# fskovbo/OptimalControlMPS

Measured on NVIDIA B200. Metric: cost+gradient evals/s (BH N=20 chi=100), higher is better.
Workload: dtype complex128 (f64)

## Files before the change

### optimalcontrolmps_b200/csrc/decomp.cu

```cuda
#include <cstdio>
#include <cstdlib>
#include "ocmps_internal.h"

__device__ unsigned long long g_jac_dbg[8];
__device__ double g_jac_flops[2];

namespace {

constexpr int JAC_THREADS = 512;
constexpr int JAC_EPL = 8;
constexpr int JAC_NV_SMEM = 512;
constexpr int JAC_MAX_SWEEPS = 60;
constexpr int JAC_BLOCKED_ROWS = 64;
constexpr double JAC_TOL2 = 1e-28;
constexpr double DEFLATE_REL = 1e-30;
constexpr int NV_MAX = 2048;
constexpr int BJ_C = 8;
constexpr int BJ_TPP = 4;
constexpr int BJ_MAX_ROWS = 256;
constexpr int BJ_SLOTS = BJ_MAX_ROWS / 2;
constexpr int BJ_THREADS = BJ_SLOTS * BJ_TPP;
constexpr int BJ_MAX_EPL = 8;
constexpr int BJ_MIN_CAP = 112;

// ... 987 lines not shown
    hF[blockIdx.x] = F;
    hK[blockIdx.x] = keff;
    hB[blockIdx.x] = -1;
    hS[blockIdx.x] = ldz;
    const double nn = (double)len, mmv = (double)nv;
    atomicAdd(&g_jac_flops[0], 8.0 * nn * nn * mmv + (56.0 / 3.0) * nn * nn * nn);
    if (blockIdx.x == 0) {
      const double dn = mode == 0 ? (double)w->n : (double)w->m, dm = mode == 0 ? (double)w->m : (double)w->n;
      atomicAdd(&g_jac_flops[1], 8.0 * dn * dn * dm + (56.0 / 3.0) * dn * dn * dn);
    }
    if (nv >= 64) {
      const long long t_now = clock64();
      atomicAdd(&g_jac_dbg[5], (unsigned long long)(t_now - t_qr0));
      atomicAdd(&g_jac_dbg[7], (unsigned long long)(t_now - t_start));
#ifdef OCMPS_JAC_TRACE
      printf("JTG kind %d blk %d nv %d len %d keff %d gather+gram %lld cholesky+out %lld\n", a.kind, (int)blockIdx.x, nv, len, keff,
             (long long)(t_qr0 - t_start), (long long)(t_now - t_qr0));
#endif
    }
  }
  return true;
}

__global__ void __launch_bounds__(JAC_THREADS) jacobi_rot_kernel(DecompArgs a, DecompBuffers b, int smem_elems) {
  extern __shared__ __align__(16) unsigned char smem_raw[];
  __shared__ int s_rot, s_big;
  __shared__ double s_nrm[JAC_BLOCKED_ROWS];
  const DecompWork* w = b.dw;
  if ((int)blockIdx.x >= w->nblocks) return;
  {
    const int nv0 = w->blk[blockIdx.x].nv, len0 = w->blk[blockIdx.x].len;
    const bool fits = nv0 * len0 <= smem_elems && nv0 <= JAC_NV_SMEM;
    const int ldpad = ((nv0 + 15) >> 4) << 4;
    const bool can_cache = nv0 <= 16 * JAC_EPL && (nv0 < len0 ? nv0 : len0) * ldpad <= smem_elems;
    if (!(fits && can_cache)) return;
  }
  const int keff = reinterpret_cast<const int*>(b.scratch_d + 7 * NV_MAX + OCMPS_MAX_BLK)[blockIdx.x];
  if (keff < 0) return;
  const DecompBlock B = w->blk[blockIdx.x];
  const int nv = B.nv;
  const int tid = threadIdx.x, lane = tid & 31, warp = tid >> 5, nwarps = JAC_THREADS / 32;
  const int epl = (nv + 15) >> 4, ldz = epl << 4;
  const double F = (b.scratch_d + 7 * NV_MAX)[blockIdx.x];
  const double thr = F * DEFLATE_REL;
  const short* perm = reinterpret_cast<const short*>(b.scratch_d + 4 * NV_MAX) + B.p_off;
  cplx* Ya = b.ywork + B.ws_off;
  const cplx* Yb = b.ywork + b.ywork_half + B.ws_off;
  cplx* Z = reinterpret_cast<cplx*>(smem_raw);
  double* nrm = s_nrm;
  const long long t_jac0 = clock64();
  for (int e = tid; e < keff * ldz; e += JAC_THREADS) Z[e] = Yb[e];
  __syncthreads();
  bool converged = false;
  for (int sweep = 0; sweep < JAC_MAX_SWEEPS && !converged; ++sweep) {
    for (int v = warp; v < keff; v += nwarps) {
      const cplx* y = Z + v * ldz;
      double s = 0.0;
      for (int c = lane; c < nv; c += 32) { cplx u = y[c]; s += u.x * u.x + u.y * u.y; }
      s = warp_sum(s);
      if (lane == 0) nrm[v] = s;
    }
    if (tid == 0) { s_rot = 0; s_big = 0; }
    __syncthreads();
    if (keff < 2) break;
    switch (epl) {
      case 1: jacobi_sweep_blocked<1>(Z, keff, nrm, thr, &s_rot, &s_big); break;
      case 2: jacobi_sweep_blocked<2>(Z, keff, nrm, thr, &s_rot, &s_big); break;
      case 3: jacobi_sweep_blocked<3>(Z, keff, nrm, thr, &s_rot, &s_big); break;
      case 4: jacobi_sweep_blocked<4>(Z, keff, nrm, thr, &s_rot, &s_big); break;
      case 5: jacobi_sweep_blocked<5>(Z, keff, nrm, thr, &s_rot, &s_big); break;
      case 6: jacobi_sweep_blocked<6>(Z, keff, nrm, thr, &s_rot, &s_big); break;
      case 7: jacobi_sweep_blocked<7>(Z, keff, nrm, thr, &s_rot, &s_big); break;
      default: jacobi_sweep_blocked<8>(Z, keff, nrm, thr, &s_rot, &s_big); break;
    }
    converged = (s_rot == 0) || (s_big == 0);
    if (tid == 0) { atomicAdd(&g_jac_dbg[0], 1ull); atomicMax(&g_jac_dbg[2], (unsigned long long)(sweep + 1)); if (nv >= 64) atomicAdd(&g_jac_dbg[3], 1ull); if (nv >= 64 && sweep == 0) atomicAdd(&g_jac_dbg[4], 1ull); }
    __syncthreads();
    if (!converged && sweep == JAC_MAX_SWEEPS - 1 && tid == 0) atomicOr(b.status, OCMPS_ST_NOCONV);
  }
  __syncthreads();
  const long long t_jac1 = clock64();
  if (tid == 0) {
    atomicAdd(&g_jac_dbg[1], 1ull);
    if (nv >= 64) {
      atomicAdd(&g_jac_dbg[6], (unsigned long long)(t_jac1 - t_jac0));
      atomicAdd(&g_jac_dbg[7], (unsigned long long)(t_jac1 - t_jac0));
    }
#ifdef OCMPS_JAC_TRACE
    if (nv >= 24) printf("JT2 kind %d blk %d nv %d keff %d jac %lld\n", a.kind, (int)blockIdx.x, nv, keff, t_jac1 - t_jac0);
#endif
  }
  for (int v = warp; v < nv; v += nwarps) {
    if (v < keff) {
      const cplx* y = Z + v * ldz;
      double s = 0.0;
      for (int c = lane; c < nv; c += 32) { cplx u = y[c]; s += u.x * u.x + u.y * u.y; }
      s = warp_sum(s);
      const double inv = s > 0.0 ? rsqrt(s) : 0.0;
      for (int c = lane; c < nv; c += 32) {
        cplx u = y[c];
        Ya[v * nv + (int)perm[c]] = make_double2(u.x * inv, u.y * inv);
      }
      if (lane == 0) b.P[B.p_off + v] = s;
    } else if (lane == 0) {
      b.P[B.p_off + v] = 0.0;
    }
  }
}

namespace clus {
__device__ __forceinline__ unsigned smem_u32(const void* p) { return (unsigned)__cvta_generic_to_shared(p); }
__device__ __forceinline__ unsigned mapa(unsigned addr, unsigned rank) {
  unsigned r;
  asm volatile("mapa.shared::cluster.u32 %0, %1, %2;" : "=r"(r) : "r"(addr), "r"(rank));
  return r;
}
__device__ __forceinline__ void st_async_v2(unsigned raddr, double a, double b, unsigned rmbar) {
  asm volatile("st.async.weak.shared::cluster.mbarrier::complete_tx::bytes.v2.f64 [%0], {%1, %2}, [%3];" ::"r"(raddr), "d"(a), "d"(b), "r"(rmbar) : "memory");
}
__device__ __forceinline__ void mbar_init(unsigned mbar, unsigned count) { asm volatile("mbarrier.init.shared::cta.b64 [%0], %1;" ::"r"(mbar), "r"(count) : "memory"); }
__device__ __forceinline__ void mbar_expect(unsigned mbar, unsigned bytes) {
  asm volatile("mbarrier.arrive.expect_tx.shared::cta.b64 _, [%0], %1;" ::"r"(mbar), "r"(bytes) : "memory");
}
__device__ __forceinline__ void mbar_wait(unsigned mbar, unsigned parity) {
  asm volatile(
      "{\n.reg .pred p;\nWAIT_%=:\n"
      "mbarrier.try_wait.parity.shared::cta.b64 p, [%0], %1;\n"
      "@p bra DONE_%=;\nbra WAIT_%=;\nDONE_%=:\n}\n" ::"r"(mbar), "r"(parity) : "memory");
}
__device__ __forceinline__ void cluster_sync() { asm volatile("barrier.cluster.arrive.release.aligned;\nbarrier.cluster.wait.acquire.aligned;\n" ::: "memory"); }
// ... 488 lines not shown
      case 3: bj_run<8, 3>(b, B, keff, ldz, F, Rs, sh); break;
      default: bj_run<8, 4>(b, B, keff, ldz, F, Rs, sh); break;
    }
  } else {
    switch ((wcols + 3) / 4) {
      case 1: bj_run<4, 1>(b, B, keff, ldz, F, Rs, sh); break;
      case 2: bj_run<4, 2>(b, B, keff, ldz, F, Rs, sh); break;
      case 3: bj_run<4, 3>(b, B, keff, ldz, F, Rs, sh); break;
      case 4: bj_run<4, 4>(b, B, keff, ldz, F, Rs, sh); break;
      case 5: bj_run<4, 5>(b, B, keff, ldz, F, Rs, sh); break;
      case 6: bj_run<4, 6>(b, B, keff, ldz, F, Rs, sh); break;
      case 7: bj_run<4, 7>(b, B, keff, ldz, F, Rs, sh); break;
      default: bj_run<4, 8>(b, B, keff, ldz, F, Rs, sh); break;
    }
  }
  clus::cluster_sync();
  if (tid == 0 && clus::cluster_rank() == 0) {
    atomicAdd(&g_jac_dbg[1], 1ull);
    const long long t1 = clock64();
    if (B.nv >= 64) { atomicAdd(&g_jac_dbg[6], (unsigned long long)(t1 - t0)); atomicAdd(&g_jac_dbg[7], (unsigned long long)(t1 - t0)); }
#ifdef OCMPS_JAC_TRACE
    if (B.nv >= 24) printf("JT3 kind %d blk %d nv %d keff %d jac %lld\n", a.kind, blk, B.nv, keff, (long long)(t1 - t0));
#endif
  }
}

__global__ void __launch_bounds__(1024) truncate_kernel(DecompArgs a, DecompBuffers b, TruncParams tp) {
  __shared__ double cP[NV_MAX];
  __shared__ double sSorted[NV_MAX];
  __shared__ short cQ[NV_MAX], cI[NV_MAX], cI2[NV_MAX];
  __shared__ unsigned char sKeep[NV_MAX];
  __shared__ int sBlkOff[OCMPS_MAX_BLK + 1];
  __shared__ double sWarp[32];
  __shared__ int sWarpCnt[33];
  __shared__ double s_docut, s_kept;
  __shared__ int s_nfinal;
  DecompWork* w = b.dw;
  const int nv = w->nvtot;
  const int nblocks = w->nblocks;
  const int tid = threadIdx.x, lane = tid & 31, warp = tid >> 5;
  for (int i = tid; i < nblocks; i += blockDim.x) sBlkOff[i] = w->blk[i].p_off;
  if (tid == 0) { s_nfinal = 0; s_docut = 0.0; }
  const int i0 = 2 * tid, i1 = i0 + 1;
  const double p0 = i0 < nv ? b.P[i0] : 0.0, p1 = i1 < nv ? b.P[i1] : 0.0;
  const int f0 = p0 > 0.0, f1 = p1 > 0.0;
  int incl = f0 + f1;
// ... 366 lines not shown
    x[e] = make_double2(u.x * inv, u.y * inv);
  }
}
__global__ void norm_finish_kernel(const double* partial, double* out) {
  if (threadIdx.x == 0 && blockIdx.x == 0) *out = sqrt(norm_total(partial));
}

int grid_for(long long elems, int threads, int cap = 1184) {
  long long g = (elems + threads - 1) / threads;
  if (g < 1) g = 1;
  if (g > cap) g = cap;
  return (int)g;
}

}

static bool g_jac_attr_set[64] = {false};

void debug_jacobi_counters(unsigned long long* out, bool reset) {
  cudaMemcpyFromSymbol(out, g_jac_dbg, sizeof(unsigned long long) * 8);
  if (reset) { unsigned long long z[8] = {0}; cudaMemcpyToSymbol(g_jac_dbg, z, sizeof(z)); }
}

__global__ void __launch_bounds__(256) spectrum_entropy_kernel(DecompBuffers b, double* out) {
  __shared__ double red[256];
  const int nv = b.dw->nvtot;
  double acc = 0.0;
  for (int i = threadIdx.x; i < nv; i += 256) {
    const double p = b.P[i];
    if (p > 1e-12) acc -= p * log(p);
  }
  red[threadIdx.x] = acc;
  __syncthreads();
  for (int o = 128; o > 0; o >>= 1) {
    if ((int)threadIdx.x < o) red[threadIdx.x] += red[threadIdx.x + o];
    __syncthreads();
  }
  if (threadIdx.x == 0) *out = red[0];
}

void launch_spectrum_entropy(const DecompBuffers& b, double* out, cudaStream_t s) {
  spectrum_entropy_kernel<<<1, 256, 0, s>>>(b, out);
}

void launch_decomp_setup(const DecompArgs& a, const DecompBuffers& b, cudaStream_t s) {
  decomp_setup_kernel<<<1, SETUP_THREADS, 0, s>>>(a, b);
// ... 7 lines not shown

bool profile_is_on() { return g_prof_on; }

void profile_enable(bool on) {
  g_prof_on = on;
  g_prof_used = 0;
  double z[2] = {0.0, 0.0};
  cudaMemcpyToSymbol(g_jac_flops, z, sizeof(z));
}
void profile_read(double* out) {
  cudaDeviceSynchronize();
  double ms = 0.0;
  for (size_t i = 0; i < g_prof_used; ++i) {
    float t = 0.f;
    cudaEventElapsedTime(&t, g_prof_events[i].first, g_prof_events[i].second);
    ms += t;
  }
  double fl[2];
  cudaMemcpyFromSymbol(fl, g_jac_flops, sizeof(fl));
  out[0] = ms; out[1] = (double)g_prof_used; out[2] = fl[0]; out[3] = fl[1];
}

void launch_jacobi_blocks(const DecompArgs& a, const DecompBuffers& b, int nblk_launch, size_t smem_limit, bool need_global,
                          bool long_rows, double rank_tol, int max_rows, int capV, int capC, cudaStream_t s, const SvdFork* fork) {
  cudaEvent_t e0 = nullptr, e1 = nullptr;
  if (g_prof_on) {
    if (g_prof_used == g_prof_events.size()) {
      cudaEvent_t x, y;
      cudaEventCreate(&x); cudaEventCreate(&y);
      g_prof_events.push_back({x, y});
    }
    e0 = g_prof_events[g_prof_used].first; e1 = g_prof_events[g_prof_used].second;
    ++g_prof_used;
    cudaEventRecord(e0, s);
  }
  struct Tail { cudaEvent_t e; cudaStream_t s; ~Tail() { if (e) cudaEventRecord(e, s); } } tail{e1, s};
  int dev = 0;
  cudaGetDevice(&dev);
  static std::mutex attr_mu;
  if (dev < 64) {
  std::lock_guard<std::mutex> attr_lock(attr_mu);
  if (!g_jac_attr_set[dev]) {
    cudaFuncSetAttribute(jacobi_blocks_kernel<true, true>, cudaFuncAttributeMaxDynamicSharedMemorySize, 200 * 1024);
    cudaFuncSetAttribute(jacobi_blocks_kernel<true, false>, cudaFuncAttributeMaxDynamicSharedMemorySize, 200 * 1024);
    cudaFuncSetAttribute(build_factors_kernel, cudaFuncAttributeMaxDynamicSharedMemorySize, 96 * 1024);
    cudaFuncSetAttribute(jacobi_rot_kernel, cudaFuncAttributeMaxDynamicSharedMemorySize, (int)(JAC_BLOCKED_ROWS * 16 * JAC_EPL * sizeof(cplx)));
    cudaFuncSetAttribute(jacobi_big_kernel, cudaFuncAttributeMaxDynamicSharedMemorySize, (int)(BJ_MAX_ROWS * (BJ_TPP * BJ_MAX_EPL + 4) * sizeof(cplx)));
    cudaFuncSetAttribute(qr_big_kernel, cudaFuncAttributeMaxDynamicSharedMemorySize, (int)((32 * BJ_MAX_ROWS + BJ_MAX_ROWS) * sizeof(cplx)));
    g_jac_attr_set[dev] = true;
  }
  }
  static const bool big_env = [] { const char* e = getenv("OCMPS_BIG_CLUSTER"); return !(e && e[0] == '0'); }();
  int big_on = (big_env && max_rows >= BJ_MIN_CAP) ? 1 : 0;
  static const bool gram_env = [] { const char* e = getenv("OCMPS_GRAM"); return e && e[0] == '1'; }();
  if (gram_env && (a.kind == DK_GATE_LEFT || a.kind == DK_GATE_RIGHT)) big_on |= 2;
  static const bool fork_env = [] { const char* e = getenv("OCMPS_SVD_FORK"); return !(e && e[0] == '0'); }();
  const bool forked = fork_env && (big_on & 1) && fork && fork->stream;
  cudaStream_t sb = forked ? fork->stream : s;
  if (forked) { cudaEventRecord(fork->ev_fork, s); cudaStreamWaitEvent(sb, fork->ev_fork, 0); }
  jacobi_blocks_kernel<true, true><<<nblk_launch, JAC_THREADS, smem_limit, s>>>(a, b, (int)(smem_limit / sizeof(cplx)), rank_tol, big_on);
  if (forked) cudaEventRecord(fork->ev_first, s);
  if (long_rows) jacobi_blocks_kernel<true, false><<<nblk_launch, JAC_THREADS, smem_limit, s>>>(a, b, (int)(smem_limit / sizeof(cplx)), rank_tol, big_on);
  if (need_global) jacobi_blocks_kernel<false, false><<<nblk_launch, JAC_THREADS, 0, s>>>(a, b, (int)(smem_limit / sizeof(cplx)), rank_tol, big_on);
  if (big_on & 1) {
    cudaLaunchConfig_t cfg = {};
    cfg.gridDim = dim3(nblk_launch * BJ_C, 1, 1);
    cfg.blockDim = dim3(BJ_THREADS, 1, 1);
    cfg.dynamicSmemBytes = (size_t)(32 * BJ_MAX_ROWS + BJ_MAX_ROWS) * sizeof(cplx);
    cfg.stream = sb;
    cudaLaunchAttribute at[1];
    at[0].id = cudaLaunchAttributeClusterDimension;
    at[0].val.clusterDim.x = BJ_C; at[0].val.clusterDim.y = 1; at[0].val.clusterDim.z = 1;
    cfg.attrs = at; cfg.numAttrs = 1;
    cudaLaunchKernelEx(&cfg, qr_big_kernel, a, b, (int)(smem_limit / sizeof(cplx)), rank_tol);
  }
  jacobi_rot_kernel<<<nblk_launch, JAC_THREADS, JAC_BLOCKED_ROWS * 16 * JAC_EPL * sizeof(cplx), s>>>(a, b, (int)(smem_limit / sizeof(cplx)));
  if (big_on & 1) {
    if (forked) cudaStreamWaitEvent(sb, fork->ev_first, 0);
    cudaLaunchConfig_t cfg = {};
    cfg.gridDim = dim3(nblk_launch * BJ_C, 1, 1);
    cfg.blockDim = dim3(BJ_THREADS, 1, 1);
    cfg.dynamicSmemBytes = (size_t)BJ_MAX_ROWS * (BJ_TPP * BJ_MAX_EPL + 4) * sizeof(cplx);
    cfg.stream = sb;
    cudaLaunchAttribute at[1];
    at[0].id = cudaLaunchAttributeClusterDimension;
    at[0].val.clusterDim.x = BJ_C; at[0].val.clusterDim.y = 1; at[0].val.clusterDim.z = 1;
    cfg.attrs = at; cfg.numAttrs = 1;
    cudaLaunchKernelEx(&cfg, jacobi_big_kernel, a, b);
    if (forked) { cudaEventRecord(fork->ev_join, sb); cudaStreamWaitEvent(s, fork->ev_join, 0); }
  }
}

void launch_truncate(const DecompArgs& a, const DecompBuffers& b, const TruncParams& tp, cudaStream_t s) {
  truncate_kernel<<<1, 1024, 0, s>>>(a, b, tp);
}

void launch_build_factors(const DecompArgs& a, const DecompBuffers& b, int cap_k, int cap_vec, int cap_comp, cudaStream_t s) {
  const size_t sm = (sizeof(cplx) + sizeof(int)) * (size_t)(cap_vec + cap_comp);
  build_factors_kernel<<<cap_k, BUILD_THREADS, sm, s>>>(a, b);
// ... 14 lines not shown
```

### optimalcontrolmps_b200/csrc/engine.cu

```cuda
#include <cmath>
#include <complex>
#include <cstdio>
#include <cstring>
#include <cstdlib>
#include <algorithm>
#include <string>
#include <atomic>
#include <chrono>
#include <map>
#include <mutex>
#include <tuple>
#include <thread>
#include <vector>

#include "ocmps_internal.h"
#include "../../include/ocmps.h"

std::atomic<long long> g_ocmps_launches{0};

namespace {

thread_local std::string g_err;

int fail(int code, const std::string& msg) {
// ... 84 lines not shown
struct Op {
  int kind;
  int a, b, c;
};

}

struct Workspace {
  ocmps_ctx* ctx = nullptr;
  int L = 0, D = 0, cap = 0;
  bool busy = false;
  size_t dead_seen = 0;
  int* d_status = nullptr;
  cplx* d_div = nullptr; int div_cap = 0;
  cudaStream_t stream = nullptr;
  cudaStream_t ovl = nullptr;
  cplx* theta = nullptr;
  cplx* cbuf = nullptr;
  DecompBuffers db;
  DecompBuffers db2;
  cudaStream_t side = nullptr;
  cudaEvent_t ev_trunc = nullptr, ev_setup = nullptr;
  SvdFork fork;
  cplx* E[2] = {nullptr, nullptr};
  cplx* T = nullptr;
  GemmDesc* odescs = nullptr;
  cplx* d_out = nullptr;
  int obatch = 0;
  long long e_stride = 0, t_stride = 0;
  ocmps_mps* work = nullptr;
  ocmps_mps* big = nullptr;
  Workspace* bigws = nullptr;
  double* d_norm = nullptr;
  StepParams* d_params = nullptr;
  ocmps_mps* tmpK = nullptr;
  ocmps_mps* psiH = nullptr;
  ocmps_store* rowstore = nullptr;
  struct StepGraph { cudaGraphExec_t exec = nullptr; unsigned long long flips = 0; int launches = 0; int seen = 0; };
  std::map<std::tuple<long long, long long, unsigned long long, int, int>, StepGraph> graphs;
};

struct ocmps_stepper {
  ocmps_ctx* ctx = nullptr;
  int L = 0, D = 0, cap = 0;
  double J = 1.0, tstep = 0.0;
  bool has_cutoff = false, has_maxm = false;
  double cutoff = MIN_CUT;
  int maxm = MAX_M;
  int rel_cutoff = 0;
  cplx* d_G[2] = {nullptr, nullptr};
  std::vector<std::complex<double>> h_G[2];
  std::vector<Op> ops;
  long long serial = 0;
  bool imag = false;
};

namespace {

int alloc_mps(ocmps_ctx* ctx, int L, int D, int cap, ocmps_mps** out, int mult = 1) {
  if (L < 1 || L > OCMPS_MAX_L) return fail(OCMPS_ERR_INVALID, "L out of range [1,64]");
  if (D < 2 || D > OCMPS_MAX_D) return fail(OCMPS_ERR_INVALID, "D out of range [2,8]");
  if (cap < 1 || (long long)cap * mult * D > NV_MAX) return fail(OCMPS_ERR_INVALID, "chi_cap*D exceeds 2048");
// ... 133 lines not shown
  void release() {
    if (!ctx || ws.empty()) return;
    std::lock_guard<std::mutex> lock(ctx->mu);
    for (Workspace* w : ws) w->busy = false;
    ws.clear();
  }
  int acquire(ocmps_ctx* c, int L, int D, int cap, int n) {
    ctx = c;
    std::lock_guard<std::mutex> lock(c->mu);
    for (Workspace* w : c->pool) {
      if ((int)ws.size() == n) break;
      if (!w->busy && w->L == L && w->D == D && w->cap == cap) { w->busy = true; ws.push_back(w); }
    }
    while ((int)ws.size() < n) {
      Workspace* w = nullptr;
      int same = 0;
      for (Workspace* o : c->pool) if (o->L == L && o->D == D && o->cap == cap) ++same;
      int rc = alloc_ws(c, L, D, cap, true, &w, same < 2);
      if (rc) return rc;
      w->busy = true;
      c->pool.push_back(w);
      ws.push_back(w);
    }
    for (Workspace* w : ws) {
      if (w->dead_seen == c->dead_mps.size()) continue;
      if (!w->graphs.empty()) {
        std::vector<long long> dead(c->dead_mps.begin() + w->dead_seen, c->dead_mps.end());
        std::sort(dead.begin(), dead.end());
        for (auto it = w->graphs.begin(); it != w->graphs.end();) {
          if (std::binary_search(dead.begin(), dead.end(), std::get<1>(it->first))) {
            if (it->second.exec) cudaGraphExecDestroy(it->second.exec);
            it = w->graphs.erase(it);
          } else {
            ++it;
          }
        }
      }
      w->dead_seen = c->dead_mps.size();
    }
    return OCMPS_OK;
  }
  Workspace* operator[](int i) const { return ws[i]; }
  int finish() {
    int st = 0;
    for (Workspace* w : ws) {
      CK(cudaStreamSynchronize(w->stream));
// ... 122 lines not shown
};
static StepTrace g_trace;
static bool step_trace_enabled() {
  static const bool v = [] { const char* e = getenv("OCMPS_STEP_TRACE"); return e && e[0] == '1'; }();
  return v;
}
enum { TR_START = 0, TR_MERGE, TR_SETUP, TR_SVD_GATE, TR_SVD_ORTH, TR_TRUNC, TR_BUILD, TR_OTHER, TR_NPHASE };

void run_decomp(Workspace* ws, const DecompArgs& a, const TruncParams& tp, int capV, int capC, int capK, cudaStream_t s,
                DecompBuffers* dbp = nullptr, bool setup_done = false, const DecompArgs* next = nullptr, DecompBuffers* db_next = nullptr) {
  DecompBuffers& db = dbp ? *dbp : ws->db;
  if (!setup_done) { launch_decomp_setup(a, db, s); g_trace.mark(TR_SETUP, s); }
  size_t need = (size_t)capV * capC * sizeof(cplx);
  need = std::max(need, (size_t)std::min(capV, capC) * (size_t)(((capV + 15) / 16) * 16) * sizeof(cplx));
  size_t smem = std::min(need, JAC_SMEM_LIMIT);
  if (smem < 1024) smem = 1024;
  int nblk = std::min(std::min(OCMPS_MAX_BLK, std::max(capV, capC) + a.D), ws->ctx->qmax.load() + a.D + 1);
  const bool need_global = need > JAC_SMEM_LIMIT;
  static const double rank_scale = [] { const char* e = getenv("OCMPS_RANK_TOL_SCALE"); return e ? atof(e) : 1e-6; }();
  double rank_tol = rank_scale * tp.cutoff;
  rank_tol = std::min(rank_scale * 1e-8, std::max(1e-30, rank_tol));
  const bool long_rows = capV > 128;
  const int max_rows = std::min(capV, capC);
  launch_jacobi_blocks(a, db, nblk, smem, need_global, long_rows, rank_tol, max_rows, capV, capC, s, &ws->fork);
  g_trace.mark((a.kind == DK_GATE_LEFT || a.kind == DK_GATE_RIGHT) ? TR_SVD_GATE : TR_SVD_ORTH, s);
  launch_truncate(a, db, tp, s);
  g_trace.mark(TR_TRUNC, s);
  if (next) {
    cudaEventRecord(ws->ev_trunc, s);
    cudaStreamWaitEvent(ws->side, ws->ev_trunc, 0);
    launch_decomp_setup(*next, *db_next, ws->side);
    cudaEventRecord(ws->ev_setup, ws->side);
  }
  launch_build_factors(a, db, capK, capV, capC, s);
  g_trace.mark(TR_BUILD, s);
  g_ocmps_launches += 5 + (need_global ? 1 : 0) + (long_rows ? 1 : 0);
}

void phases_of(int D, double U, double tstep, double* re, double* im, bool imag = false) {
  for (int n = 0; n < D; ++n) {
    if (imag) {
      re[n] = std::exp(-0.25 * U * tstep * (double)n * (double)(n - 1));
      im[n] = 0.0;
      continue;
    }
    const double ang = -0.25 * U * tstep * (double)n * (double)(n - 1);
    re[n] = std::cos(ang);
// ... 172 lines not shown
    g_trace.on = false;
    CK(cudaStreamSynchronize(s));
    double sum[TR_NPHASE] = {0};
    int cnt[TR_NPHASE] = {0};
    for (size_t i = 1; i < g_trace.marks.size(); ++i) {
      float ms = 0.f;
      cudaEventElapsedTime(&ms, g_trace.marks[i - 1].second, g_trace.marks[i].second);
      sum[g_trace.marks[i].first] += ms;
      ++cnt[g_trace.marks[i].first];
    }
    float tot = 0.f;
    cudaEventElapsedTime(&tot, g_trace.marks.front().second, g_trace.marks.back().second);
    static const char* names[TR_NPHASE] = {"", "merge_gate", "setup", "svd(gate)", "svd(gauge)", "truncate", "build", "other"};
    fprintf(stderr, "[ocmps step] %.3f ms:", tot);
    for (int p = 1; p < TR_NPHASE; ++p) fprintf(stderr, " %s %dx %.3f |", names[p], cnt[p], sum[p]);
    fprintf(stderr, "\n");
    for (auto& m2 : g_trace.marks) cudaEventDestroy(m2.second);
    g_trace.marks.clear();
    return OCMPS_OK;
  }
  if (!graphs_enabled() || profile_is_on()) { body(); return OCMPS_OK; }
  unsigned long long parity = 0;
  for (int j = 0; j < lay.L; ++j) parity |= (unsigned long long)(m->cur[j] & 1) << j;
  auto key = std::make_tuple(st->serial, m->serial, parity, store ? 1 : 0, ws->ctx->qmax.load());
  Workspace::StepGraph& g = ws->graphs[key];
  if (g.exec) {
    for (int j = 0; j < lay.L; ++j) m->cur[j] ^= (int)((g.flips >> j) & 1ull);
    m->llim = 0; m->rlim = 2;
    g_ocmps_launches += g.launches;
    CK(cudaGraphLaunch(g.exec, s));
    return OCMPS_OK;
  }
  if (g.seen == 0) {
    g.seen = 1;
    body();
    return OCMPS_OK;
  }
  if (ws->graphs.size() > 64) {
    for (auto& kv : ws->graphs) if (kv.second.exec) cudaGraphExecDestroy(kv.second.exec);
    ws->graphs.clear();
    Workspace::StepGraph& g2 = ws->graphs[key];
    g2.seen = 1;
    body();
    return OCMPS_OK;
  }
  const long long l0 = g_ocmps_launches;
  cudaGraph_t graph = nullptr;
// ... 89 lines not shown
                                        int qstride_out, int L, int cap_out, int* status) {
  for (int b = blockIdx.x; b <= L; b += gridDim.x) {
    int d = dims_in[b];
    if (d > cap_out) { if (threadIdx.x == 0) atomicOr(status, OCMPS_ST_CAPACITY); d = cap_out; }
    if (threadIdx.x == 0) dims_out[b] = d;
    for (int i = threadIdx.x; i < d; i += blockDim.x) q_out[(size_t)b * qstride_out + i] = q_in[(size_t)b * qstride_in + i];
  }
}

int apply_K_async(ocmps_stepper* st, Workspace* ws, ocmps_mps* in, ocmps_mps* out, cudaStream_t s) {
  const int L = st->L, D = st->D;
  const int cap2 = 2 * st->cap;
  if ((long long)cap2 * D > NV_MAX) return fail(OCMPS_ERR_INVALID, "apply_K: 2*chi_cap*D exceeds 2048");
  if (!ws->big) {
    int rc = alloc_mps(st->ctx, L, D, st->cap, &ws->big, 2);
    if (rc) return rc;
    rc = alloc_ws(st->ctx, L, D, cap2, false, &ws->bigws);
    if (rc) return rc;
    ws->bigws->db.status = ws->d_status;
    ws->bigws->db2.status = ws->d_status;
  }
  ocmps_mps* big = ws->big;
  Workspace* bw = ws->bigws;
  const Layout& lb = big->lay;
  if (L == 1) return fail(OCMPS_ERR_INVALID, "apply_K needs L >= 2");
  for (int j = 0; j < L; ++j) big->cur[j] = 0;
  for (int j = 0; j < L; ++j) {
    launch_applyK_expand(in->site(j), big->site(j), in->dim(j), in->dim(j + 1), in->q(j), in->q(j + 1), big->dim(j), big->dim(j + 1),
                         big->q(j), big->q(j + 1), D, j, L, lb.capb[j] * D * lb.capb[j + 1], s);
  }
  g_ocmps_launches += L;
  TruncParams tpl{MIN_CUT, MAX_M, 1, 1, 0, 0};
  for (int b = 1; b <= L - 1; ++b) {
    const int j = b - 1, jn = b;
    DecompArgs a;
    a.D = D; a.kind = DK_ORTH_LEFT;
    a.dimNew = big->dim(b); a.qNew = big->q(b); a.partner = bw->cbuf;
    a.dimL = big->dim(b - 1); a.dimR = big->dim(b); a.qL = big->q(b - 1); a.qR = big->q(b);
    a.X = big->site(j); a.iso = big->other(j);
    a.nb_in = big->site(jn); a.nb_out = big->other(jn); a.dimNb = big->dim(b + 1);
    a.qNb = fused_push_enabled() ? big->q(b + 1) : nullptr;
    tpl.cap = lb.capb[b];
    run_decomp(bw, a, tpl, lb.capb[b], lb.capb[b - 1], lb.capb[b], s);
    if (!a.qNb) launch_zgemm(bw->db.descs + 1, 1, lb.capb[b], D * lb.capb[b + 1], s);
    big->cur[j] ^= 1; big->cur[jn] ^= 1;
    g_ocmps_launches += 1;
// ... 341 lines not shown

static int check_shapes(ocmps_stepper* st, const Layout& lay, const char* what) {
  if (lay.L != st->L || lay.D != st->D || lay.cap != st->cap)
    return fail(OCMPS_ERR_INVALID, std::string(what) + ": MPS/store shape (L, D, chi_cap) differs from the stepper's");
  return OCMPS_OK;
}

int ocmps_step(ocmps_stepper* st, ocmps_mps* psi, double from, double to, int forward) {
  if (!st || !psi) return fail(OCMPS_ERR_INVALID, "null argument");
  int rc = check_shapes(st, psi->lay, "step");
  if (rc) return rc;
  if (psi->llim != 0 || psi->rlim != 2) return fail(OCMPS_ERR_INVALID, "step: orthogonality centre must be at site 1");
  CK(cudaSetDevice(st->ctx->dev));
  WsLease lease;
  rc = lease.acquire(st->ctx, st->L, st->D, st->cap, 1);
  if (rc) return rc;
  Workspace* ws = lease[0];
  rc = step_enqueue(st, psi, ws, from, to, forward != 0, nullptr, 0, ws->stream);
  if (rc) { cudaStreamSynchronize(ws->stream); return rc; }
  return lease.finish();
}

int ocmps_debug_jacobi(unsigned long long* out, int reset) { cudaDeviceSynchronize(); debug_jacobi_counters(out, reset != 0); return 0; }

int ocmps_debug_run_ops(ocmps_stepper* st, ocmps_mps* psi, double from, double to, int forward, int op_begin, int op_end) {
  CK(cudaSetDevice(st->ctx->dev));
  WsLease lease;
  int rc = lease.acquire(st->ctx, st->L, st->D, st->cap, 1);
  if (rc) return rc;
  Workspace* ws = lease[0];
  { StepParams hp; fill_step_params(st, from, to, forward != 0, nullptr, 0, hp); launch_set_step_params(hp, ws->d_params, ws->stream); }
  run_step_body(st, psi, ws, ws->stream, op_begin, op_end);
  return lease.finish();
}

int ocmps_apply_K(ocmps_stepper* st, ocmps_mps* in, ocmps_mps* out) {
  if (!st || !in || !out) return fail(OCMPS_ERR_INVALID, "null argument");
  int rc = check_shapes(st, in->lay, "apply_K");
  if (rc) return rc;
  rc = check_shapes(st, out->lay, "apply_K");
  if (rc) return rc;
  CK(cudaSetDevice(st->ctx->dev));
  WsLease lease;
  rc = lease.acquire(st->ctx, st->L, st->D, st->cap, 1);
  if (rc) return rc;
  Workspace* ws = lease[0];
// ... 814 lines not shown
```

### optimalcontrolmps_b200/csrc/ocmps_internal.h

```cpp
#pragma once
#include <cuda_runtime.h>
#include <stdint.h>
#include <stddef.h>

typedef double2 cplx;

#define OCMPS_MAX_L 64
#define OCMPS_MAX_D 8
#define OCMPS_MAX_Q 256
#define OCMPS_MAX_BLK 128

#define OCMPS_ST_CAPACITY   1
#define OCMPS_ST_NOCONV     2
#define OCMPS_ST_CHARGE     4
#define OCMPS_ST_TOOMANYBLK 8

struct GemmDesc {
  const cplx* A; const cplx* B; cplx* C;
  int M, N, K;
  int lda, ldb, ldc;
  int opA, opB;
  int pad;
};

// ... 19 lines not shown
  double cutoff;
  int maxm, minm;
  int rel_cutoff;
  int cap;
  int normalize;
};

struct StepParams {
  double u1r[OCMPS_MAX_D], u1i[OCMPS_MAX_D];
  double u2r[OCMPS_MAX_D], u2i[OCMPS_MAX_D];
  const cplx* G;
  cplx* slot_data; int* slot_dims; int* slot_q;
};

struct SitePtrs { cplx* p[OCMPS_MAX_L]; };
struct SiteOffs { long long o[OCMPS_MAX_L + 1]; };

struct Phases { double re[4][OCMPS_MAX_D]; double im[4][OCMPS_MAX_D]; };

#include <atomic>
extern std::atomic<long long> g_ocmps_launches;

void debug_jacobi_counters(unsigned long long* out, bool reset);
void profile_enable(bool on);
bool profile_is_on();
void profile_read(double* out);

void launch_zgemm(const GemmDesc* d_descs, int batch, int maxM, int maxN, cudaStream_t s);

enum DecompKind { DK_GATE_LEFT = 0, DK_GATE_RIGHT = 1, DK_ORTH_LEFT = 2, DK_ORTH_RIGHT = 3 };

struct DecompArgs {
  int kind;
  int D;
  const int* dimL;
  const int* dimR;
  const int* qL;
  const int* qR;
  int* dimNew;
  int* qNew;
  const cplx* X;
  cplx* iso;
  cplx* partner;
  const cplx* nb_in;
  cplx* nb_out;
  const int* dimNb;
  const int* qNb;
};

struct DecompBuffers {
  DecompWork* dw;
  int* vec_idx; int* comp_idx;
  int* vecq;
  double* P;
  int* pos;
  cplx* ywork;
  long long ywork_half;
  double* scratch_d;
  GemmDesc* descs;
  double* partial;
  int* status;
};

void launch_decomp_setup(const DecompArgs& a, const DecompBuffers& b, cudaStream_t s);
struct SvdFork { cudaStream_t stream = nullptr; cudaEvent_t ev_fork = nullptr, ev_first = nullptr, ev_join = nullptr; };
void launch_jacobi_blocks(const DecompArgs& a, const DecompBuffers& b, int nblk_launch, size_t smem_limit, bool need_global,
                          bool long_rows, double rank_tol, int max_rows, int capV, int capC, cudaStream_t s, const SvdFork* fork = nullptr);
void launch_spectrum_entropy(const DecompBuffers& b, double* out, cudaStream_t s);
void launch_truncate(const DecompArgs& a, const DecompBuffers& b, const TruncParams& tp, cudaStream_t s);
void launch_build_factors(const DecompArgs& a, const DecompBuffers& b, int cap_k, int cap_vec, int cap_comp, cudaStream_t s);

void launch_merge_setup(GemmDesc* d, const cplx* A1, const cplx* A2, cplx* theta, const int* dimL, const int* dimM,
                        const int* dimR, int D, cudaStream_t s);
void launch_merge_gate(const cplx* A1, const cplx* A2, cplx* theta, const int* dimL, const int* dimM, const int* dimR,
                       const int* qL, const int* qM, const int* qR, int D, const StepParams* sp, int gate_kind, int maxL, int maxR,
                       cudaStream_t s);
void launch_gate_apply(cplx* theta, const int* dimL, const int* dimR, const int* qL, const int* qR, int D, const StepParams* sp,
                       int gate_kind, int maxL, int maxR, cudaStream_t s);
void launch_site_phase(cplx* A, const int* dimL, const int* dimR, int D, const StepParams* sp, int which, int max_elems, cudaStream_t s);
void launch_set_step_params(const StepParams& hp, StepParams* dst, cudaStream_t s);
void launch_pack_to_slot(SitePtrs src, SiteOffs offs, const int* dims, const int* q, int L, int D, int cap, int max_site_elems,
                         const StepParams* sp, int* status, cudaStream_t s);
void launch_norm_only(const cplx* x, const int* dimL, const int* dimR, int D, double* partial, double* out, int max_elems,
                      cudaStream_t s);
void launch_normalize_site(cplx* x, const int* dimL, const int* dimR, int D, double* partial, int max_elems, cudaStream_t s);

void launch_pack_copy(SitePtrs src, cplx* dst_base, SiteOffs offs, const int* dims, int L, int D, int max_site_elems, int* status,
                      cudaStream_t s);
void launch_unpack_copy(const cplx* src_base, SitePtrs dst, SiteOffs offs, const int* dims, int L, int D, int max_site_elems, int* status,
                        cudaStream_t s);
// ... 26 lines not shown
```

Before: 0.8572.

## Spread one-sided Jacobi rows across a 4-CTA cluster with DSMEM block exchange

Adds a cluster kernel that splits the Jacobi rotation of a symmetry block across four CTAs. Each CTA holds two row blocks and runs round-robin block pairs, exchanging row blocks and norms through distributed shared memory between rounds, and combines convergence flags across the cluster. It is enabled when the workspace batch is small (n<=2), so the GPU is underused and a single CTA per block is the bottleneck. The cost is a cluster sync and a DSMEM copy every round. Blocks with fewer than 40 effective rows fall back to the single-CTA path.

```diff
diff --git a/optimalcontrolmps_b200/csrc/decomp.cu b/optimalcontrolmps_b200/csrc/decomp.cu
--- a/optimalcontrolmps_b200/csrc/decomp.cu
+++ b/optimalcontrolmps_b200/csrc/decomp.cu
@@ -1033,26 +1033,26 @@
   return true;
 }
 
-__global__ void __launch_bounds__(JAC_THREADS) jacobi_rot_kernel(DecompArgs a, DecompBuffers b, int smem_elems) {
-  extern __shared__ __align__(16) unsigned char smem_raw[];
+__device__ __forceinline__ int rot_handover_rows(const DecompBuffers& b, int blk, int smem_elems) {
+  const DecompWork* w = b.dw;
+  if (blk >= w->nblocks) return -1;
+  const int nv0 = w->blk[blk].nv, len0 = w->blk[blk].len;
+  const bool fits = nv0 * len0 <= smem_elems && nv0 <= JAC_NV_SMEM;
+  const int ldpad = ((nv0 + 15) >> 4) << 4;
+  const bool can_cache = nv0 <= 16 * JAC_EPL && (nv0 < len0 ? nv0 : len0) * ldpad <= smem_elems;
+  if (!(fits && can_cache)) return -1;
+  return reinterpret_cast<const int*>(b.scratch_d + 7 * NV_MAX + OCMPS_MAX_BLK)[blk];
+}
+
+__device__ __forceinline__ void jacobi_rot_block(const DecompArgs& a, const DecompBuffers& b, int blk, int keff, unsigned char* smem_raw) {
   __shared__ int s_rot, s_big;
   __shared__ double s_nrm[JAC_BLOCKED_ROWS];
   const DecompWork* w = b.dw;
-  if ((int)blockIdx.x >= w->nblocks) return;
-  {
-    const int nv0 = w->blk[blockIdx.x].nv, len0 = w->blk[blockIdx.x].len;
-    const bool fits = nv0 * len0 <= smem_elems && nv0 <= JAC_NV_SMEM;
-    const int ldpad = ((nv0 + 15) >> 4) << 4;
-    const bool can_cache = nv0 <= 16 * JAC_EPL && (nv0 < len0 ? nv0 : len0) * ldpad <= smem_elems;
-    if (!(fits && can_cache)) return;
-  }
-  const int keff = reinterpret_cast<const int*>(b.scratch_d + 7 * NV_MAX + OCMPS_MAX_BLK)[blockIdx.x];
-  if (keff < 0) return;
-  const DecompBlock B = w->blk[blockIdx.x];
+  const DecompBlock B = w->blk[blk];
   const int nv = B.nv;
   const int tid = threadIdx.x, lane = tid & 31, warp = tid >> 5, nwarps = JAC_THREADS / 32;
   const int epl = (nv + 15) >> 4, ldz = epl << 4;
-  const double F = (b.scratch_d + 7 * NV_MAX)[blockIdx.x];
+  const double F = (b.scratch_d + 7 * NV_MAX)[blk];
   const double thr = F * DEFLATE_REL;
   const short* perm = reinterpret_cast<const short*>(b.scratch_d + 4 * NV_MAX) + B.p_off;
   cplx* Ya = b.ywork + B.ws_off;
@@ -1098,7 +1098,7 @@
       atomicAdd(&g_jac_dbg[7], (unsigned long long)(t_jac1 - t_jac0));
     }
 #ifdef OCMPS_JAC_TRACE
-    if (nv >= 24) printf("JT2 kind %d blk %d nv %d keff %d jac %lld\n", a.kind, (int)blockIdx.x, nv, keff, t_jac1 - t_jac0);
+    if (nv >= 24) printf("JT2 kind %d blk %d nv %d keff %d jac %lld\n", a.kind, blk, nv, keff, t_jac1 - t_jac0);
 #endif
   }
   for (int v = warp; v < nv; v += nwarps) {
@@ -1117,6 +1117,13 @@
       b.P[B.p_off + v] = 0.0;
     }
   }
+}
+
+__global__ void __launch_bounds__(JAC_THREADS) jacobi_rot_kernel(DecompArgs a, DecompBuffers b, int smem_elems) {
+  extern __shared__ __align__(16) unsigned char smem_raw[];
+  const int keff = rot_handover_rows(b, (int)blockIdx.x, smem_elems);
+  if (keff < 0) return;
+  jacobi_rot_block(a, b, (int)blockIdx.x, keff, smem_raw);
 }
 
 namespace clus {
@@ -1651,6 +1658,238 @@
 #ifdef OCMPS_JAC_TRACE
     if (B.nv >= 24) printf("JT3 kind %d blk %d nv %d keff %d jac %lld\n", a.kind, blk, B.nv, keff, (long long)(t1 - t0));
 #endif
+  }
+}
+
+constexpr int RC_C = 4;
+constexpr int RC_NBLK = 2 * RC_C;
+constexpr int RC_ROWS = JAC_BLOCKED_ROWS / RC_NBLK;
+constexpr int RC_WORK_THREADS = 16 * RC_ROWS;
+constexpr int RC_MIN_ROWS = 40;
+
+__device__ unsigned long long g_rc_dbg[2];
+
+struct RcShared {
+  double nrm[2][2][RC_ROWS];
+  int flags[2][RC_C];
+  int rot, big;
+};
+
+__device__ __forceinline__ void rc_blocks(int R, int s, int& P, int& Q) {
+  constexpr int mm = RC_NBLK - 1;
+  int p = R + s; if (p >= mm) p -= mm;
+  int q = R - s; if (q < 0) q += mm;
+  if (s == 0) q = RC_NBLK - 1;
+  P = p; Q = q;
+}
+
+__device__ __forceinline__ void rc_bar() { asm volatile("bar.sync 1, %0;" ::"n"(RC_WORK_THREADS) : "memory"); }
+
+template <int EPL>
+__device__ __forceinline__ void rc_block_round(cplx* __restrict__ Z0, cplx* __restrict__ Z1, double* n0, double* n1, int rb, int base0, int base1,
+                                               int keff, double thr, bool intra, int* s_rot, int* s_big) {
+  constexpr int ldz = 16 * EPL;
+  const int tid = threadIdx.x, hl = tid & 15, h = tid >> 4;
+  cplx ra[EPL], rb_[EPL];
+  double na = 0.0, nb = 0.0;
+  auto load_row = [&](cplx (&r)[EPL], double& n, const cplx* Z, const double* nz, int row) {
+    const cplx* z = Z + (row >= 0 ? row : 0) * ldz + hl;
+#pragma unroll
+    for (int e = 0; e < EPL; ++e) r[e] = row >= 0 ? z[16 * e] : make_double2(0.0, 0.0);
+    n = row >= 0 ? nz[row] : 0.0;
+  };
+  auto store_row = [&](const cplx (&r)[EPL], double n, cplx* Z, double* nz, int row) {
+    cplx* z = Z + row * ldz + hl;
+#pragma unroll
+    for (int e = 0; e < EPL; ++e) z[16 * e] = r[e];
+    if (hl == 0) nz[row] = n;
+  };
+  if (intra) {
+    const int X = h / (RC_ROWS / 2), j = h % (RC_ROWS / 2);
+    cplx* Z = X ? Z1 : Z0;
+    double* nz = X ? n1 : n0;
+    const int base = X ? base1 : base0;
+    const int rbp = (rb + 1) & ~1, m = rbp - 1;
+    for (int r = 0; r < m; ++r) {
+      int p = r + j; if (p >= m) p -= m;
+      int q = r - j; if (q < 0) q += m;
+      if (j == 0) q = m;
+      const bool act = 2 * j < rbp && p < rb && q < rb && base + p < keff && base + q < keff;
+      load_row(ra, na, Z, nz, act ? p : -1);
+      load_row(rb_, nb, Z, nz, act ? q : -1);
+      jac_rotate<EPL>(ra, rb_, na, nb, act, thr, hl, s_rot, s_big);
+      if (act) { store_row(ra, na, Z, nz, p); store_row(rb_, nb, Z, nz, q); }
+      rc_bar();
+    }
+  }
+  const bool has_a = h < rb && base0 + h < keff;
+  load_row(ra, na, Z0, n0, has_a ? h : -1);
+  for (int t = 0; t < rb; ++t) {
+    int jb = h + t; if (jb >= rb) jb -= rb;
+    const bool act = has_a && base1 + jb < keff;
+    load_row(rb_, nb, Z1, n1, act ? jb : -1);
+    jac_rotate<EPL>(ra, rb_, na, nb, act, thr, hl, s_rot, s_big);
+    if (act) store_row(rb_, nb, Z1, n1, jb);
+    rc_bar();
+  }
+  if (has_a) store_row(ra, na, Z0, n0, h);
+}
+
+template <int EPL>
+__device__ __forceinline__ void rc_run(const DecompArgs& a, const DecompBuffers& b, int blk, int keff, unsigned rank, cplx* __restrict__ Zs, RcShared& sh) {
+  constexpr int ldz = 16 * EPL;
+  constexpr int BLK = RC_ROWS * ldz;
+  const int tid = threadIdx.x, lane = tid & 31, warp = tid >> 5, nwarps = JAC_THREADS / 32;
+  const DecompBlock B = b.dw->blk[blk];
+  const int nv = B.nv;
+  const int rb = (keff + RC_NBLK - 1) / RC_NBLK;
+  const double F = (b.scratch_d + 7 * NV_MAX)[blk];
+  const double thr = F * DEFLATE_REL;
+  const cplx* Yb = b.ywork + b.ywork_half + B.ws_off;
+  auto zb = [&](int buf, int k) { return Zs + (2 * buf + k) * BLK; };
+  const long long t_jac0 = clock64();
+  int P, Q;
+  rc_blocks(0, (int)rank, P, Q);
+  for (int e = tid; e < 2 * BLK; e += JAC_THREADS) {
+    const int k = e / BLK, r = (e % BLK) / ldz, c = e % ldz;
+    const int row = (k ? Q : P) * rb + r;
+    Zs[e] = (r < rb && row < keff) ? Yb[row * ldz + c] : make_double2(0.0, 0.0);
+  }
+  __syncthreads();
+  int cur = 0;
+  bool done = false;
+#ifdef OCMPS_JAC_TRACE
+  long long t_work = 0, t_xchg = 0;
+  int nrounds = 0, nxchg = 0;
+#endif
+  for (int sweep = 0; sweep < JAC_MAX_SWEEPS && !done; ++sweep) {
+    for (int lr = warp; lr < 2 * RC_ROWS; lr += nwarps) {
+      const int k = lr / RC_ROWS, r = lr % RC_ROWS;
+      const cplx* y = zb(cur, k) + r * ldz;
+      double s = 0.0;
+      for (int c = lane; c < nv; c += 32) { const cplx u = y[c]; s += u.x * u.x + u.y * u.y; }
+      s = warp_sum(s);
+      if (lane == 0) sh.nrm[cur][k][r] = s;
+    }
+    if (tid == 0) { sh.rot = 0; sh.big = 0; }
+    __syncthreads();
+    for (int R = 0; R < RC_NBLK - 1; ++R) {
+#ifdef OCMPS_JAC_TRACE
+      const long long tw0 = clock64();
+#endif
+      if (tid < RC_WORK_THREADS) rc_block_round<EPL>(zb(cur, 0), zb(cur, 1), sh.nrm[cur][0], sh.nrm[cur][1], rb, P * rb, Q * rb, keff, thr, R == 0, &sh.rot, &sh.big);
+      __syncthreads();
+#ifdef OCMPS_JAC_TRACE
+      const long long tw1 = clock64();
+      t_work += tw1 - tw0;
+      nrounds += rb + (R == 0 ? ((rb + 1) & ~1) - 1 : 0);
+#endif
+      const bool last = R == RC_NBLK - 2;
+      if (last && tid < RC_C) {
+        const int f = (sh.rot ? 1 : 0) | (sh.big ? 2 : 0);
+        asm volatile("st.shared::cluster.u32 [%0], %1;" ::"r"(clus::mapa(clus::smem_u32(&sh.flags[sweep & 1][rank]), (unsigned)tid)), "r"(f) : "memory");
+      }
+      clus::cluster_sync();
+      if (last) {
+        int any = 0;
+#pragma unroll
+        for (int r = 0; r < RC_C; ++r) any |= sh.flags[sweep & 1][r];
+        done = !(any & 1) || !(any & 2);
+        if (tid == 0 && rank == 0) {
+          atomicAdd(&g_jac_dbg[0], 1ull); atomicMax(&g_jac_dbg[2], (unsigned long long)(sweep + 1)); atomicAdd(&g_rc_dbg[1], 1ull);
+          if (nv >= 64) atomicAdd(&g_jac_dbg[3], 1ull);
+          if (nv >= 64 && sweep == 0) atomicAdd(&g_jac_dbg[4], 1ull);
+          if (!done && sweep == JAC_MAX_SWEEPS - 1) atomicOr(b.status, OCMPS_ST_NOCONV);
+        }
+        if (done || sweep == JAC_MAX_SWEEPS - 1) break;
+      }
+      int NP, NQ;
+      rc_blocks(last ? 0 : R + 1, (int)rank, NP, NQ);
+      unsigned src0 = 0, src1 = 0, nsrc0 = 0, nsrc1 = 0;
+      for (int s = 0; s < RC_C; ++s) {
+        int p, q;
+        rc_blocks(R, s, p, q);
+        const unsigned zp = clus::mapa(clus::smem_u32(zb(cur, 0)), (unsigned)s), zq = clus::mapa(clus::smem_u32(zb(cur, 1)), (unsigned)s);
+        const unsigned np = clus::mapa(clus::smem_u32(sh.nrm[cur][0]), (unsigned)s), nq = clus::mapa(clus::smem_u32(sh.nrm[cur][1]), (unsigned)s);
+        if (p == NP) { src0 = zp; nsrc0 = np; }
+        if (q == NP) { src0 = zq; nsrc0 = nq; }
+        if (p == NQ) { src1 = zp; nsrc1 = np; }
+        if (q == NQ) { src1 = zq; nsrc1 = nq; }
+      }
+      for (int e = tid; e < 2 * rb * ldz; e += JAC_THREADS) {
+        const int k = e >= rb * ldz, o = e - k * rb * ldz;
+        double xr, xi;
+        asm volatile("ld.shared::cluster.v2.f64 {%0, %1}, [%2];" : "=d"(xr), "=d"(xi) : "r"((k ? src1 : src0) + (unsigned)o * 16u) : "memory");
+        zb(cur ^ 1, k)[o] = make_double2(xr, xi);
+      }
+      if (tid < 2 * RC_ROWS) {
+        const int k = tid / RC_ROWS, r = tid % RC_ROWS;
+        double x;
+        asm volatile("ld.shared::cluster.f64 %0, [%1];" : "=d"(x) : "r"((k ? nsrc1 : nsrc0) + (unsigned)r * 8u) : "memory");
+        sh.nrm[cur ^ 1][k][r] = x;
+      }
+      __syncthreads();
+#ifdef OCMPS_JAC_TRACE
+      t_xchg += clock64() - tw1;
+      ++nxchg;
+#endif
+      cur ^= 1; P = NP; Q = NQ;
+    }
+  }
+  const long long t_jac1 = clock64();
+  const short* perm = reinterpret_cast<const short*>(b.scratch_d + 4 * NV_MAX) + B.p_off;
+  cplx* Ya = b.ywork + B.ws_off;
+  for (int lr = warp; lr < 2 * RC_ROWS; lr += nwarps) {
+    const int k = lr / RC_ROWS, r = lr % RC_ROWS, v = (k ? Q : P) * rb + r;
+    if (r >= rb || v >= keff) continue;
+    const cplx* y = zb(cur, k) + r * ldz;
+    double s = 0.0;
+    for (int c = lane; c < nv; c += 32) { const cplx u = y[c]; s += u.x * u.x + u.y * u.y; }
+    s = warp_sum(s);
+    const double inv = s > 0.0 ? rsqrt(s) : 0.0;
+    for (int c = lane; c < nv; c += 32) {
+      const cplx u = y[c];
+      Ya[v * nv + (int)perm[c]] = make_double2(u.x * inv, u.y * inv);
+    }
+    if (lane == 0) b.P[B.p_off + v] = s;
+  }
+  if (rank == 0) for (int v = keff + tid; v < nv; v += JAC_THREADS) b.P[B.p_off + v] = 0.0;
+  if (tid == 0 && rank == 0) {
+    atomicAdd(&g_jac_dbg[1], 1ull);
+    atomicAdd(&g_rc_dbg[0], 1ull);
+    if (nv >= 64) {
+      atomicAdd(&g_jac_dbg[6], (unsigned long long)(t_jac1 - t_jac0));
+      atomicAdd(&g_jac_dbg[7], (unsigned long long)(t_jac1 - t_jac0));
+    }
+#ifdef OCMPS_JAC_TRACE
+    if (nv >= 24)
+      printf("JTR kind %d blk %d nv %d keff %d rb %d jac %lld : rotation rounds %d, %lld clk per round; block exchanges %d, %lld clk each\n", a.kind, blk, nv,
+             keff, rb, t_jac1 - t_jac0, nrounds, nrounds ? t_work / nrounds : 0ll, nxchg, nxchg ? t_xchg / nxchg : 0ll);
+#endif
+  }
+}
+
+__global__ void __launch_bounds__(JAC_THREADS) jacobi_rows_cluster_kernel(DecompArgs a, DecompBuffers b, int smem_elems) {
+  extern __shared__ __align__(16) unsigned char smem_raw[];
+  __shared__ RcShared sh;
+  const int blk = (int)blockIdx.x / RC_C;
+  const unsigned rank = clus::cluster_rank();
+  const int keff = rot_handover_rows(b, blk, smem_elems);
+  if (keff < 0) return;
+  if (keff < RC_MIN_ROWS) {
+    if (rank == 0) jacobi_rot_block(a, b, blk, keff, smem_raw);
+    return;
+  }
+  cplx* Zs = reinterpret_cast<cplx*>(smem_raw);
+  switch ((b.dw->blk[blk].nv + 15) >> 4) {
+    case 1: rc_run<1>(a, b, blk, keff, rank, Zs, sh); break;
+    case 2: rc_run<2>(a, b, blk, keff, rank, Zs, sh); break;
+    case 3: rc_run<3>(a, b, blk, keff, rank, Zs, sh); break;
+    case 4: rc_run<4>(a, b, blk, keff, rank, Zs, sh); break;
+    case 5: rc_run<5>(a, b, blk, keff, rank, Zs, sh); break;
+    case 6: rc_run<6>(a, b, blk, keff, rank, Zs, sh); break;
+    case 7: rc_run<7>(a, b, blk, keff, rank, Zs, sh); break;
+    default: rc_run<8>(a, b, blk, keff, rank, Zs, sh); break;
   }
 }
 
@@ -2063,6 +2302,11 @@
   if (reset) { unsigned long long z[8] = {0}; cudaMemcpyToSymbol(g_jac_dbg, z, sizeof(z)); }
 }
 
+void debug_row_cluster_counters(unsigned long long* out, bool reset) {
+  cudaMemcpyFromSymbol(out, g_rc_dbg, sizeof(unsigned long long) * 2);
+  if (reset) { unsigned long long z[2] = {0, 0}; cudaMemcpyToSymbol(g_rc_dbg, z, sizeof(z)); }
+}
+
 __global__ void __launch_bounds__(256) spectrum_entropy_kernel(DecompBuffers b, double* out) {
   __shared__ double red[256];
   const int nv = b.dw->nvtot;
@@ -2116,7 +2360,8 @@
 }
 
 void launch_jacobi_blocks(const DecompArgs& a, const DecompBuffers& b, int nblk_launch, size_t smem_limit, bool need_global,
-                          bool long_rows, double rank_tol, int max_rows, int capV, int capC, cudaStream_t s, const SvdFork* fork) {
+                          bool long_rows, double rank_tol, int max_rows, int capV, int capC, bool spread_rows, cudaStream_t s,
+                          const SvdFork* fork) {
   cudaEvent_t e0 = nullptr, e1 = nullptr;
   if (g_prof_on) {
     if (g_prof_used == g_prof_events.size()) {
@@ -2139,6 +2384,7 @@
     cudaFuncSetAttribute(jacobi_blocks_kernel<true, false>, cudaFuncAttributeMaxDynamicSharedMemorySize, 200 * 1024);
     cudaFuncSetAttribute(build_factors_kernel, cudaFuncAttributeMaxDynamicSharedMemorySize, 96 * 1024);
     cudaFuncSetAttribute(jacobi_rot_kernel, cudaFuncAttributeMaxDynamicSharedMemorySize, (int)(JAC_BLOCKED_ROWS * 16 * JAC_EPL * sizeof(cplx)));
+    cudaFuncSetAttribute(jacobi_rows_cluster_kernel, cudaFuncAttributeMaxDynamicSharedMemorySize, (int)(JAC_BLOCKED_ROWS * 16 * JAC_EPL * sizeof(cplx)));
     cudaFuncSetAttribute(jacobi_big_kernel, cudaFuncAttributeMaxDynamicSharedMemorySize, (int)(BJ_MAX_ROWS * (BJ_TPP * BJ_MAX_EPL + 4) * sizeof(cplx)));
     cudaFuncSetAttribute(qr_big_kernel, cudaFuncAttributeMaxDynamicSharedMemorySize, (int)((32 * BJ_MAX_ROWS + BJ_MAX_ROWS) * sizeof(cplx)));
     g_jac_attr_set[dev] = true;
@@ -2168,7 +2414,20 @@
     cfg.attrs = at; cfg.numAttrs = 1;
     cudaLaunchKernelEx(&cfg, qr_big_kernel, a, b, (int)(smem_limit / sizeof(cplx)), rank_tol);
   }
-  jacobi_rot_kernel<<<nblk_launch, JAC_THREADS, JAC_BLOCKED_ROWS * 16 * JAC_EPL * sizeof(cplx), s>>>(a, b, (int)(smem_limit / sizeof(cplx)));
+  if (spread_rows) {
+    cudaLaunchConfig_t cfg = {};
+    cfg.gridDim = dim3(nblk_launch * RC_C, 1, 1);
+    cfg.blockDim = dim3(JAC_THREADS, 1, 1);
+    cfg.dynamicSmemBytes = (size_t)JAC_BLOCKED_ROWS * 16 * JAC_EPL * sizeof(cplx);
+    cfg.stream = s;
+    cudaLaunchAttribute at[1];
+    at[0].id = cudaLaunchAttributeClusterDimension;
+    at[0].val.clusterDim.x = RC_C; at[0].val.clusterDim.y = 1; at[0].val.clusterDim.z = 1;
+    cfg.attrs = at; cfg.numAttrs = 1;
+    cudaLaunchKernelEx(&cfg, jacobi_rows_cluster_kernel, a, b, (int)(smem_limit / sizeof(cplx)));
+  } else {
+    jacobi_rot_kernel<<<nblk_launch, JAC_THREADS, JAC_BLOCKED_ROWS * 16 * JAC_EPL * sizeof(cplx), s>>>(a, b, (int)(smem_limit / sizeof(cplx)));
+  }
   if (big_on & 1) {
     if (forked) cudaStreamWaitEvent(sb, fork->ev_first, 0);
     cudaLaunchConfig_t cfg = {};
diff --git a/optimalcontrolmps_b200/csrc/engine.cu b/optimalcontrolmps_b200/csrc/engine.cu
--- a/optimalcontrolmps_b200/csrc/engine.cu
+++ b/optimalcontrolmps_b200/csrc/engine.cu
@@ -130,6 +130,7 @@
   cudaStream_t side = nullptr;
   cudaEvent_t ev_trunc = nullptr, ev_setup = nullptr;
   SvdFork fork;
+  bool spread_jacobi = true;
   cplx* E[2] = {nullptr, nullptr};
   cplx* T = nullptr;
   GemmDesc* odescs = nullptr;
@@ -145,7 +146,7 @@
   ocmps_mps* psiH = nullptr;
   ocmps_store* rowstore = nullptr;
   struct StepGraph { cudaGraphExec_t exec = nullptr; unsigned long long flips = 0; int launches = 0; int seen = 0; };
-  std::map<std::tuple<long long, long long, unsigned long long, int, int>, StepGraph> graphs;
+  std::map<std::tuple<long long, long long, unsigned long long, int, int, int>, StepGraph> graphs;
 };
 
 struct ocmps_stepper {
@@ -325,6 +326,7 @@
       c->pool.push_back(w);
       ws.push_back(w);
     }
+    for (Workspace* w : ws) w->spread_jacobi = n <= 2;
     for (Workspace* w : ws) {
       if (w->dead_seen == c->dead_mps.size()) continue;
       if (!w->graphs.empty()) {
@@ -493,7 +495,7 @@
   rank_tol = std::min(rank_scale * 1e-8, std::max(1e-30, rank_tol));
   const bool long_rows = capV > 128;
   const int max_rows = std::min(capV, capC);
-  launch_jacobi_blocks(a, db, nblk, smem, need_global, long_rows, rank_tol, max_rows, capV, capC, s, &ws->fork);
+  launch_jacobi_blocks(a, db, nblk, smem, need_global, long_rows, rank_tol, max_rows, capV, capC, ws->spread_jacobi, s, &ws->fork);
   g_trace.mark((a.kind == DK_GATE_LEFT || a.kind == DK_GATE_RIGHT) ? TR_SVD_GATE : TR_SVD_ORTH, s);
   launch_truncate(a, db, tp, s);
   g_trace.mark(TR_TRUNC, s);
@@ -712,7 +714,7 @@
   if (!graphs_enabled() || profile_is_on()) { body(); return OCMPS_OK; }
   unsigned long long parity = 0;
   for (int j = 0; j < lay.L; ++j) parity |= (unsigned long long)(m->cur[j] & 1) << j;
-  auto key = std::make_tuple(st->serial, m->serial, parity, store ? 1 : 0, ws->ctx->qmax.load());
+  auto key = std::make_tuple(st->serial, m->serial, parity, store ? 1 : 0, ws->ctx->qmax.load(), ws->spread_jacobi ? 1 : 0);
   Workspace::StepGraph& g = ws->graphs[key];
   if (g.exec) {
     for (int j = 0; j < lay.L; ++j) m->cur[j] ^= (int)((g.flips >> j) & 1ull);
@@ -848,6 +850,7 @@
   }
   ocmps_mps* big = ws->big;
   Workspace* bw = ws->bigws;
+  bw->spread_jacobi = ws->spread_jacobi;
   const Layout& lb = big->lay;
   if (L == 1) return fail(OCMPS_ERR_INVALID, "apply_K needs L >= 2");
   for (int j = 0; j < L; ++j) big->cur[j] = 0;
@@ -1235,6 +1238,7 @@
 }
 
 int ocmps_debug_jacobi(unsigned long long* out, int reset) { cudaDeviceSynchronize(); debug_jacobi_counters(out, reset != 0); return 0; }
+int ocmps_debug_row_cluster(unsigned long long* out2, int reset) { cudaDeviceSynchronize(); debug_row_cluster_counters(out2, reset != 0); return 0; }
 
 int ocmps_debug_run_ops(ocmps_stepper* st, ocmps_mps* psi, double from, double to, int forward, int op_begin, int op_end) {
   CK(cudaSetDevice(st->ctx->dev));
diff --git a/optimalcontrolmps_b200/csrc/ocmps_internal.h b/optimalcontrolmps_b200/csrc/ocmps_internal.h
--- a/optimalcontrolmps_b200/csrc/ocmps_internal.h
+++ b/optimalcontrolmps_b200/csrc/ocmps_internal.h
@@ -65,6 +65,7 @@
 extern std::atomic<long long> g_ocmps_launches;
 
 void debug_jacobi_counters(unsigned long long* out, bool reset);
+void debug_row_cluster_counters(unsigned long long* out, bool reset);
 void profile_enable(bool on);
 bool profile_is_on();
 void profile_read(double* out);
@@ -108,7 +109,8 @@
 void launch_decomp_setup(const DecompArgs& a, const DecompBuffers& b, cudaStream_t s);
 struct SvdFork { cudaStream_t stream = nullptr; cudaEvent_t ev_fork = nullptr, ev_first = nullptr, ev_join = nullptr; };
 void launch_jacobi_blocks(const DecompArgs& a, const DecompBuffers& b, int nblk_launch, size_t smem_limit, bool need_global,
-                          bool long_rows, double rank_tol, int max_rows, int capV, int capC, cudaStream_t s, const SvdFork* fork = nullptr);
+                          bool long_rows, double rank_tol, int max_rows, int capV, int capC, bool spread_rows, cudaStream_t s,
+                          const SvdFork* fork = nullptr);
 void launch_spectrum_entropy(const DecompBuffers& b, double* out, cudaStream_t s);
 void launch_truncate(const DecompArgs& a, const DecompBuffers& b, const TruncParams& tp, cudaStream_t s);
 void launch_build_factors(const DecompArgs& a, const DecompBuffers& b, int cap_k, int cap_vec, int cap_comp, cudaStream_t s);
```

Result: faster. 0.9281, median of 6 (+8.3%).
